# b0nefish/tiler

Hardware: AMD Instinct MI355X
Metric: FrameTiling Mtiles/sec @1080p 8×8, 64k tileset; % HBM roofline at 1/2/4/8 GPU (higher is better)
Workload: dtype f32

## Files before the change

include/tiler_ann.h:

```cpp
#ifndef TILER_ANN_H
#define TILER_ANN_H

#include <stdint.h>

#ifdef __cplusplus
extern "C" {
#endif

typedef struct ann_kdtree ann_kdtree;

ann_kdtree *ann_kdtree_create(float **pa, int n, int dd, int bs, int split);
void ann_kdtree_destroy(ann_kdtree *akd);
int ann_kdtree_search(ann_kdtree *akd, float *q, float eps, float *err);
int ann_kdtree_pri_search(ann_kdtree *akd, float *q, float eps, float *err);
int ann_kdtree_search_multi(ann_kdtree *akd, int *idxs, float *errs, int cnt, float *q, float eps);

#define TILER_SPLIT_ANN_KD_STD 0
#define TILER_SPLIT_INDEX_ORDER 100

ann_kdtree *ann_kdtree_create_dev(const float *d_rows, int n, int dd, void *stream);
ann_kdtree *ann_kdtree_create_dev_ex(const float *d_rows, int n, int dd, int bs, int split, void *stream);

int ann_kdtree_search_batch(ann_kdtree *akd, const float *q, int nq, float eps, int *idx, float *err);
int ann_kdtree_search_multi_batch(ann_kdtree *akd, const float *q, int nq, int k, float eps, int *idxs, float *errs);
int ann_kdtree_pri_search_batch(ann_kdtree *akd, const float *q, int nq, float eps, int *idx, float *err);
int ann_kdtree_search_batch_dev(ann_kdtree *akd, const float *d_q, int nq, int k, int *d_idx, float *d_err,
                                void *stream);

typedef struct {
    int64_t queries;
    int64_t fallback_queries;
    int64_t exhaustive_queries;
    int32_t exact_integer;
    int32_t splits;
    int64_t orbit_groups;
    int32_t orbit_search;
    int32_t orbit_ksteps;
    int64_t orbit_expansions;
    int64_t orbit_rescored;
    int32_t tie_order;
    int32_t kd_levels;
    double kd_build_ms;
    int64_t kd_replayed;
    int64_t flat_queries;
    int64_t searched_queries;
    int64_t searched_flat_queries;
    int64_t dup_queries;
} tiler_search_stats;
int ann_kdtree_get_stats(ann_kdtree *akd, tiler_search_stats *out);
int tiler_set_scan_limits(int max_k1, int max_k8);
int tiler_debug_force_replay(int on);
int tiler_debug_pri_outcomes(ann_kdtree *akd, int64_t out[3]);
int tiler_debug_shortlist_gate(int on);
int tiler_debug_ft_dedup(int mode);
int tiler_combine_stats(ann_kdtree *akd, int64_t *calls, int64_t *batches, int32_t *max_batch);
int tiler_debug_percall_bench(ann_kdtree *akd, const float *q, int nq, int k, int threads, int32_t *idx, float *err,
                              double *wall_s, double *lone_us);
int tiler_kdtree_positions(ann_kdtree *akd, int32_t *pos);

#define TILER_ALL_DEVICES (-1)
int tiler_init(int device);
int tiler_device_count(void);
int tiler_kdtree_device(ann_kdtree *akd);
int tiler_kdtree_replicate(ann_kdtree *akd, int device);
int tiler_placement_plan(int ndev, const int64_t *bytes, int n, int32_t *dev_out);
int tiler_debug_force_replicas(int on);
int tiler_shutdown(void);
const char *tiler_last_error(void);
int tiler_set_gamma(double g0, double g1);
int tiler_timing_enable(int on);
double tiler_timing_get(const char *kernel, int *launches);
int tiler_timing_reset(void);

int tiler_psyv_batch(int n, const int32_t *rgb, int n_tiles, const uint8_t *palpix, const int32_t *tile_of, int n_palettes,
                     const int32_t *palettes,
                     const int32_t *pal_of, const uint8_t *flags_per, int flags, int gamma, double *out64, float *out32);
int tiler_psyv_batch_dev(int n, const int32_t *rgb, const uint8_t *palpix, const int32_t *tile_of,
                         const int32_t *palettes, const int32_t *pal_of, const uint8_t *flags_per, int flags, int gamma,
                         double *out64, float *out32, void *stream);
int tiler_psyv_batch_ps(int n, const int32_t *rgb, int n_tiles, const uint8_t *palpix, const int32_t *tile_of,
                        int n_palettes, int palsize, const int32_t *palettes, const int32_t *pal_of,
                        const uint8_t *flags_per, int flags, int gamma, double *out64, float *out32);
int tiler_psyv_batch_ps_dev(int n, const int32_t *rgb, const uint8_t *palpix, const int32_t *tile_of,
                            const int32_t *palettes, int palsize, const int32_t *pal_of, const uint8_t *flags_per,
                            int flags, int gamma, double *out64, float *out32, void *stream);
int tiler_debug_psyv_lane_items(int64_t min_items);

// ... 268 lines not shown
```

tiler_amd/_lib.py:

```python
from __future__ import annotations

import ctypes
import os
import re

_HERE = os.path.dirname(os.path.abspath(__file__))
LIB_PATH = os.path.join(_HERE, "lib", "libANN.so")
_DEFAULT_LIB_PATH = LIB_PATH
HEADER_PATH = os.path.join(os.path.dirname(_HERE), "include", "tiler_ann.h")

c_int = ctypes.c_int
c_long = ctypes.c_long
c_float = ctypes.c_float
c_double = ctypes.c_double
c_void_p = ctypes.c_void_p
c_char_p = ctypes.c_char_p
c_size_t = ctypes.c_size_t
c_uint32 = ctypes.c_uint32
P = ctypes.POINTER


class TilerError(RuntimeError):
    pass

# ... 21 lines not shown
    _fields_ = [("tile", c_void_p), ("pal", c_void_p), ("hm", c_void_p), ("vm", c_void_p), ("smoothed", c_void_p),
                ("palpix", c_void_p), ("thm", c_void_p), ("tvm", c_void_p), ("palettes", c_void_p),
                ("kf_start", c_void_p), ("frames", ctypes.c_int64), ("positions", ctypes.c_int64),
                ("tiles", ctypes.c_int64), ("keyframes", ctypes.c_int32), ("n_palettes", ctypes.c_int32),
                ("palsize", ctypes.c_int32), ("first_keyframe", ctypes.c_int32), ("width", ctypes.c_int32),
                ("height", ctypes.c_int32), ("fps", c_double)]


class PrepareInfo(ctypes.Structure):
    _fields_ = [("items", ctypes.c_int64), ("candidates", ctypes.c_int64)]


_SIGS = {
    "ann_kdtree_create": (c_void_p, [P(P(c_float)), c_int, c_int, c_int, c_int]),
    "ann_kdtree_create_dev": (c_void_p, [c_void_p, c_int, c_int, c_void_p]),
    "ann_kdtree_create_dev_ex": (c_void_p, [c_void_p, c_int, c_int, c_int, c_int, c_void_p]),
    "tiler_kdtree_positions": (c_int, [c_void_p, c_void_p]),
    "ann_kdtree_destroy": (None, [c_void_p]),
    "ann_kdtree_search": (c_int, [c_void_p, c_void_p, c_float, c_void_p]),
    "ann_kdtree_pri_search": (c_int, [c_void_p, c_void_p, c_float, c_void_p]),
    "ann_kdtree_search_multi": (c_int, [c_void_p, c_void_p, c_void_p, c_int, c_void_p, c_float]),
    "ann_kdtree_search_batch": (c_int, [c_void_p, c_void_p, c_int, c_float, c_void_p, c_void_p]),
    "ann_kdtree_search_multi_batch": (c_int, [c_void_p, c_void_p, c_int, c_int, c_float, c_void_p, c_void_p]),
    "ann_kdtree_pri_search_batch": (c_int, [c_void_p, c_void_p, c_int, c_float, c_void_p, c_void_p]),
    "ann_kdtree_search_batch_dev": (c_int, [c_void_p, c_void_p, c_int, c_int, c_void_p, c_void_p, c_void_p]),
    "ann_kdtree_get_stats": (c_int, [c_void_p, P(SearchStats)]),
    "tiler_set_scan_limits": (c_int, [c_int, c_int]),
    "tiler_debug_percall_bench": (c_int, [c_void_p, c_void_p, c_int, c_int, c_int, c_void_p, c_void_p, P(c_double),
                                          P(c_double)]),
    "tiler_debug_force_replay": (c_int, [c_int]),
    "tiler_debug_pri_outcomes": (c_int, [c_void_p, P(ctypes.c_int64)]),
    "tiler_debug_shortlist_gate": (c_int, [c_int]),
    "tiler_debug_ft_dedup": (c_int, [c_int]),
    "tiler_combine_stats": (c_int, [c_void_p, P(ctypes.c_int64), P(ctypes.c_int64), P(ctypes.c_int32)]),
    "tiler_init": (c_int, [c_int]),
    "tiler_device_count": (c_int, []),
    "tiler_kdtree_device": (c_int, [c_void_p]),
    "tiler_kdtree_replicate": (c_int, [c_void_p, c_int]),
    "tiler_placement_plan": (c_int, [c_int, c_void_p, c_int, c_void_p]),
    "tiler_debug_force_replicas": (c_int, [c_int]),
    "tiler_shutdown": (c_int, []),
    "tiler_last_error": (c_char_p, []),
    "tiler_set_gamma": (c_int, [c_double, c_double]),
    "tiler_timing_enable": (c_int, [c_int]),
    "tiler_timing_get": (c_double, [c_char_p, P(c_int)]),
    "tiler_timing_reset": (c_int, []),
    "tiler_psyv_batch": (c_int, [c_int, c_void_p, c_int, c_void_p, c_void_p, c_int, c_void_p, c_void_p, c_void_p,
                                 c_int, c_int, c_void_p, c_void_p]),
    "tiler_psyv_batch_dev": (c_int, [c_int, c_void_p, c_void_p, c_void_p, c_void_p, c_void_p, c_void_p, c_int, c_int,
                                     c_void_p, c_void_p, c_void_p]),
    "tiler_psyv_batch_ps": (c_int, [c_int, c_void_p, c_int, c_void_p, c_void_p, c_int, c_int, c_void_p, c_void_p,
                                    c_void_p, c_int, c_int, c_void_p, c_void_p]),
    "tiler_psyv_batch_ps_dev": (c_int, [c_int, c_void_p, c_void_p, c_void_p, c_void_p, c_int, c_void_p, c_void_p,
                                        c_int, c_int, c_void_p, c_void_p, c_void_p]),
    "tiler_ft_set_maps": (c_int, [c_void_p, c_void_p, c_void_p, c_void_p]),
    "tiler_ft_get_maps": (c_int, [c_void_p, c_void_p, c_void_p, c_void_p]),
    "tiler_prepare_frame_tiling_dev": (c_void_p, [c_void_p, c_void_p, c_void_p, ctypes.c_int64, c_void_p, c_void_p,
                                                  c_void_p, c_int, c_void_p, c_int, c_int, c_void_p, c_int, c_int,
                                                  c_void_p, P(PrepareInfo)]),
    "tiler_prepare_frame_tiling_ps_dev": (c_void_p, [c_void_p, c_void_p, c_void_p, ctypes.c_int64, c_void_p,
                                                     c_void_p, c_void_p, c_int, c_void_p, c_int, c_int, c_int,
                                                     c_void_p, c_int, c_int, c_void_p, P(PrepareInfo)]),
    "tiler_frame_tiling": (c_int, [c_void_p, c_void_p, c_int, c_int, c_int, c_void_p, c_void_p, c_void_p, c_void_p,
                                   c_void_p]),
    "tiler_frame_tiling_dev": (c_int, [c_void_p, c_void_p, c_int, c_int, c_int, c_void_p, c_void_p, c_void_p,
                                       c_void_p, c_void_p, c_void_p]),
# ... 181 lines not shown
```

tiler_amd/csrc/ann_api.hip:

```cpp
#include <float.h>
#include <math.h>
#include <string.h>

#include <atomic>
#include <algorithm>
#include <chrono>
#include <thread>
#include <condition_variable>
#include <deque>
#include <mutex>
#include <string>
#include <vector>

#include "../../include/tiler_ann.h"
#include "dither.hpp"
#include "gtm_write.hpp"
#include "palette.hpp"
#include "play.hpp"
#include "prepare.hpp"
#include "kmeans.hpp"
#include "detmath.hpp"
#include "keyframes.hpp"
#include "load.hpp"
#include "scale.hpp"
// ... 950 lines not shown
int ann_kdtree_search_multi(ann_kdtree *t, int *idxs, float *errs, int cnt, float *q, float eps) {
    (void)eps;
    return combined_search(t, q, cnt, idxs, errs);
}

int tiler_set_scan_limits(int max_k1, int max_k8) {
    if (max_k1 < 0 || max_k8 < 0) {
        set_error("tiler_set_scan_limits: negative limit");
        return -1;
    }
    nn_set_scan_limits(max_k1, max_k8);
    return 0;
}

int tiler_debug_force_replay(int on) {
    nn_set_force_replay(on);
    return 0;
}

int tiler_debug_shortlist_gate(int on) {
    nn_set_shortlist_gate(on);
    return 0;
}

int tiler_debug_ft_dedup(int mode) {
    if (mode < 0 || mode > 2) {
        set_error("tiler_debug_ft_dedup: mode must be 0, 1 or 2");
        return -1;
    }
    nn_set_ft_dedup(mode);
    return 0;
}

int tiler_combine_stats(ann_kdtree *t, int64_t *calls, int64_t *batches, int32_t *max_batch) {
    if (!t) {
        set_error("tiler_combine_stats: null handle");
        return -1;
    }
    std::lock_guard<std::mutex> lk(t->comb.m);
    if (calls) *calls = t->comb.calls;
    if (batches) *batches = t->comb.batches;
    if (max_batch) *max_batch = t->comb.max_batch;
    return 0;
}

int tiler_debug_percall_bench(ann_kdtree *t, const float *q, int nq, int k, int threads, int32_t *idx, float *err,
                              double *wall_s, double *lone_us) {
    if (!t || !t->ix || nq < 0 || (nq > 0 && (!q || !idx || !err)) || k < 1 || k > 32 || threads < 1 || threads > 256) {
        set_error("tiler_debug_percall_bench: invalid arguments");
        return -1;
    }
    const int d = t->ix->d;
    auto call = [&](int i) -> int {
        float *qi = const_cast<float *>(q + (size_t)i * d);
        if (k == 1) {
            const int r = ann_kdtree_search(t, qi, 0.0f, err + i);
            idx[i] = r;
            return r < 0 && t->ix->n > 0 ? -1 : 0;
        }
        return ann_kdtree_search_multi(t, idx + (size_t)i * k, err + (size_t)i * k, k, qi, 0.0f);
    };
    const int nl = std::min(nq, 64);
    std::vector<double> lat;
    for (int i = 0; i < nl; i++) {
        const auto a = std::chrono::steady_clock::now();
        if (call(i)) return -1;
// ... 999 lines not shown
```

tiler_amd/csrc/frame_tiling.hip:

```cpp
#include "frame_tiling.hpp"

#include <atomic>

#include "nn_search.hpp"
#include "orbit.hpp"
#include "psyv.hpp"

namespace tiler {

__global__ __launch_bounds__(256) void ft_flat_flag_kernel(const int32_t *__restrict__ rgb, int Q, uint8_t *flag,
                                                           int *bcnt) {
    const long i = (long)blockIdx.x * 256 + threadIdx.x;
    int other = 0;
    if (i < Q) {
        const int4 *t = reinterpret_cast<const int4 *>(rgb + i * 64);
        const int c0 = rgb[i * 64];
        bool flat = true;
#pragma unroll
        for (int k = 0; k < 16; k++) {
            const int4 v = t[k];
            flat = flat && v.x == c0 && v.y == c0 && v.z == c0 && v.w == c0;
        }
        flag[i] = flat ? 1 : 0;
        other = flat ? 0 : 1;
// ... 264 lines not shown
            }
            TILER_HIP_CHECK(hipStreamSynchronize(stream));
            const int U = f.h_cnt[0] + f.h_cnt[1];
            if (U < 1 || U > Q) {
                set_error("frame tiling: inconsistent representative count");
                return -1;
            }
            engaged = U <= Q - Q / 8;
            if (engaged) {
                nq = U;
                rep_of = f.drep;
            } else if (group) {
                cnt = f.fcnt + 2;
                place(nullptr, f.fbcnt + (size_t)2 * nb, nullptr, cnt);
            }
        } else {
            hipLaunchKernelGGL(ft_flat_flag_kernel, dim3(nb), dim3(256), 0, stream, d_rgb, Q, f.fflag, f.fbcnt);
            hipLaunchKernelGGL(ft_flat_scan_kernel, dim3(1), dim3(1024), 0, stream, f.fbcnt, nb, f.fcnt);
            place(nullptr, f.fbcnt, nullptr, cnt);
        }
        TILER_HIP_CHECK(hipGetLastError());
        if (engaged || group) {
            perm = f.fperm;
            if (group) flat_cnt = cnt;
        }
    }

    FtMaps fm;
    if (maps) fm = perm ? FtMaps{f.ftile, f.fpal, f.fhm, f.fvm} : *maps;
    SearchOpts so;
    so.rootbox_ready = fuse_rb;
    so.orbit_prepared = orbit;
    so.flat_cnt = flat_cnt;
    const float *box = fuse_rb ? ix->kd->d_box : nullptr;
    float *rootbox = fuse_rb ? ix->scratch.kd_rootbox : nullptr;
    if (orbit) {
        if (orbit_ft_queries(ix, d_rgb, nq, gamma, f.qrows, box, rootbox, stream, perm)) return -1;
    } else {
        PsyvArgs pa;
        pa.n = nq;
        pa.rgb = d_rgb;
        pa.perm = perm;
        pa.flags = use_wavelets ? PSYV_WAVELETS : 0;
        pa.gamma = gamma;
        pa.out32 = f.qrows;
        pa.box = box;
        pa.rootbox = rootbox;
        if (launch_psyv(pa, stream)) return -1;
    }
    if (nn_search_dev(ix, f.qrows, nq, 1, perm ? f.fidx : d_idx, perm ? f.ferr : d_err, maps ? &fm : nullptr, stream, so))
        return -1;
    if (!perm) return 0;
    if (rep_of) {
        ix->last.queries = Q;
        ix->last.dup = Q - nq;
        ix->last.ft_nonflat = f.h_cnt[2];
    }
    KTimer tm(rep_of ? "ft_dedup" : nullptr, stream);
    hipLaunchKernelGGL(ft_output_kernel, dim3(nb), dim3(256), 0, stream, Q, rep_of, (const int *)f.dpos,
                       (const int *)f.fidx, (const float *)f.ferr, (const int32_t *)f.ftile, (const int32_t *)f.fpal,
                       (const uint8_t *)f.fhm, (const uint8_t *)f.fvm, d_idx, d_err, maps ? *maps : FtMaps{});
    TILER_HIP_CHECK(hipGetLastError());
    return 0;
}

}
// ... 1 lines not shown
```

tiler_amd/csrc/nn_search.hip:

```cpp
#include <float.h>
#include <math.h>
#include <stdlib.h>
#include <string.h>

#include <algorithm>
#include <atomic>

#include "nn_search.hpp"
#include "kdorder_dev.hpp"
#include "nn_dev.hpp"
#include "orbit.hpp"
#include "orbit_map_gen.hpp"

#pragma clang fp contract(off)

namespace tiler {

enum { QF_INT = 1, QF_BAD = 2 };

struct PrepArgs {
    const float *rows;
    long n;
    int d, S;
    float scale;
// ... 1726 lines not shown
    TILER_HIP_CHECK(hipGetLastError());
    return 0;
}

static int search_core(NNIndex *ix, RescoreArgs &ra, const float *d_q, int nq, int k, hipStream_t stream,
                       const SearchOpts &opt) {
    if (scan_small_takes(ix, nq, k)) return scan_small(ix, ra, nq, k, stream);
    const bool mfma = ix->S > 0 && k <= 8;
    if (!mfma) {
        ix->last.splits = 0;
        ix->last.fallback = nq;
        ra.tq.ex_list = nullptr;
        return launch_exact(ra, nq, std::min(nq, 4096), stream);
    }
    const int v16 = ix->S16 > 0 ? SL16_L : 0;
    const int L = v16 ? v16 : 8;
    const int lpq = v16 ? 4 : 2;
    const int nblk = v16 ? ix->nblk16 : ix->nblk;
    const int max_split = 64 / (lpq * L);
    const int qpwg = v16 ? SL16_NW * SL16_QB * 16 : (ix->S == 12 ? 512 : ix->S == 4 ? 32 * gen_qb_s4(nq) * GEN_NW_S4 : 256);
    const int wgs = (nq + qpwg - 1) / qpwg;
    int nsplit = std::max(1, std::min(max_split, (1024 + wgs - 1) / wgs));
    nsplit = std::min(nsplit, nblk);
    const int bps = (nblk + nsplit - 1) / nsplit;
    nsplit = (nblk + bps - 1) / bps;
    ix->last.splits = nsplit;
    if (ensure_scratch(ix, nq, (long)nq * nsplit * lpq * L)) return -1;
    SearchScratch &s = ix->scratch;
    TILER_HIP_CHECK(hipMemsetAsync(s.fb_count, 0, 16, stream));
    ix->last_orbit = 0;
    ra.tq = TierQueues{s.fb_list, s.fb_count, s.ex_list, s.fb_count + 1, nq, s.thr};
    ra.qstat = s.qstat;
    if (k == 1 && ix->orbit) {
        const OrbitTail t{ra.tq, ra.kd, ra.out, s.t2best, opt.flat_cnt, nullptr};
        if (orbit_search(ix, d_q, nq, t, stream, opt.orbit_prepared && k == 1)) return -1;
        ix->last_orbit = 1;
        return search_tail(ix, ra, nq, stream, &t);
    }
    const long nqblk = (nq + 31) / 32;
    PrepArgs pa{d_q, nq, ix->d, ix->S, ix->scale, (half8 *)s.qfrag, nullptr, nullptr, s.qstat, nullptr, 0};
    {
        KTimer t_prep("nn_prep", stream);
        hipLaunchKernelGGL(prep_rows_kernel, dim3((unsigned)std::min<long>(4096, (nqblk + 3) / 4)), dim3(256), 0,
                           stream, pa);
    }
    TILER_HIP_CHECK(hipGetLastError());
    if (v16) {
        Prep16Args p16{d_q, nq, ix->d, ix->S16, ix->scale, (half8 *)s.qfrag16, nullptr, 0, ix->d == 192 ? 1 : 0};
        {
            KTimer t_prep("nn_prep", stream);
            hipLaunchKernelGGL(prep16_kernel, dim3((unsigned)std::min<long>(4096, ((nq + 15) / 16 + 3) / 4)),
                               dim3(256), 0, stream, p16);
        }
        TILER_HIP_CHECK(hipGetLastError());
        {
            if (launch_shortlist16<6, SL16_L>(ix, nq, nsplit, bps, k == 1 && g_gate16.load(std::memory_order_relaxed),
                                         opt.flat_cnt, stream))
                return -1;
        }
    } else if (dispatch_shortlist<8>(ix, nq, nsplit, bps, stream)) {
        return -1;
    }
    ra.key = s.key;
    ra.idx = s.idx;
    ra.L = L;
    ra.lpq = lpq;
    ra.nsplit = nsplit;
// ... 42 lines not shown
```

tiler_amd/csrc/nn_search.hpp:

```cpp
#pragma once
#include <mutex>
#include <vector>

#include "frame_tiling.hpp"
#include "kdtree.hpp"
#include "tiler_common.hpp"

namespace tiler {

struct DsStat {
    unsigned long long max_n2_bits;
    unsigned long long max_h2_bits;
    unsigned long long max_e2_bits;
    unsigned long long max_abs_bits;
    unsigned int not_int;
    unsigned int bad;
    unsigned int pad[2];
};

struct QStat {
    double n2;
    double hn;
    double en;
    int flags;
// ... 6 lines not shown
    void *qfrag = nullptr;
    QStat *qstat = nullptr;
    float *key = nullptr;
    int *idx = nullptr;
    int *fb_list = nullptr;
    int *fb_count = nullptr;
    void *qfrag16 = nullptr;
    float *thr = nullptr;
    float2 *gate = nullptr;
    int *ex_list = nullptr;
    int *ccnt = nullptr;
    int *cbuf = nullptr;
    unsigned long long *t2best = nullptr;
    int *kd_list = nullptr;
    int *kd_count = nullptr;
    float *kd_rootbox = nullptr;
    uint8_t *kd_done = nullptr;
    size_t cap_q = 0, cap_keys = 0;
};

struct TierQueues {
    int *fb_list, *fb_count;
    int *ex_list, *ex_count;
    int fb_max;
    float *thr;
};

struct LastSearch {
    long long queries = 0, fallback = 0;
    int splits = 0;
    const int *flat_dev = nullptr;
    long flat_nq = 0, flat_qpw = 0, flat_wgs = 0;
    long long searched = 0, dup = 0, ft_nonflat = -1;
};

struct NNIndex {
    int n = 0, d = 0, S = 0, nblk = 0;
    float scale = 1.0f;
    double maxN = 0, maxH = 0, maxE = 0, max_abs = 0;
    bool exact_int = false;
    int perm = 0;
    float *d_rows = nullptr;
    float *d_rowsT = nullptr;
    void *d_frag = nullptr;
    float *d_nc = nullptr;
    float *d_seed = nullptr;
    int S16 = 0, nblk16 = 0;
    void *d_frag16 = nullptr;
    float *d_seed16 = nullptr;
    int32_t *d_tr_tile = nullptr, *d_tr_pal = nullptr;
    uint8_t *d_tr_attr = nullptr;
    SearchScratch scratch;
    std::mutex mu;
    LastSearch last;
    FtScratch ft;
    hipEvent_t done_event = nullptr;
    int last_orbit = 0;
    OrbitIndex *orbit = nullptr;
    KdTree *kd = nullptr;
    int bs = 1, split = KD_SPLIT_STD;
    int *h_fb_count = nullptr;
};

NNIndex *nn_index_create_dev(float *d_rows, int n, int d, int bs, int split, hipStream_t stream);
void nn_index_destroy(NNIndex *ix);
void nn_scratch_free(SearchScratch &s, bool synced = false);
bool nn_search_is_small(const NNIndex *ix, int nq, int k);

struct FtMaps {
    int32_t *tile = nullptr, *pal = nullptr;
    uint8_t *hm = nullptr, *vm = nullptr;
};

struct SearchOpts {
    bool rootbox_ready = false;
    bool orbit_prepared = false;
    const int *flat_cnt = nullptr;
    int *h_idx = nullptr;
    float *h_err = nullptr;
};

int nn_search_dev(NNIndex *ix, const float *d_q, int nq, int k, int *d_idx, float *d_err, const FtMaps *maps,
                  hipStream_t stream, const SearchOpts &opt = SearchOpts());
int nn_ensure_rootbox(NNIndex *ix, int nq);
bool nn_generic_takes_flat(const NNIndex *ix);

void nn_set_scan_limits(int max_k1, int max_k8);
void nn_set_force_replay(int on);
void nn_set_shortlist_gate(int on);

}
```

tiler_amd/csrc/orbit.hip:

```cpp
#include <float.h>
#include <math.h>
#include <string.h>

#include <algorithm>
#include <vector>

#include "kdorder_dev.hpp"
#include "nn_dev.hpp"
#include "psyv_dev.hpp"
#include "orbit.hpp"
#include "orbit_map_gen.hpp"

namespace tiler {

static constexpr int OD = 192;
static constexpr int OS = 12;
#ifndef ORB_XBATCH
#define ORB_XBATCH 3
#endif
#ifndef ORB_RS_WAVES
#define ORB_RS_WAVES 6
#endif
#ifndef ORB_STG_ROWS
#define ORB_STG_ROWS 4
#endif
#ifndef ORB_PR_UNROLL
#define ORB_PR_UNROLL 8
#endif
#ifndef ORB_DU
#define ORB_DU 4
#endif

struct OrbitMap {
    int16_t src[OD][4];
    float w[OD][4];
    float cs[OD], qs[OD];
    int16_t msrc[3][OD];
// ... 381 lines not shown
            t_bd |= bad;
        }
    }
    if (dataset) {
        __shared__ double r_d[ORB_PW][4];
        __shared__ int r_b[ORB_PW];
        const double mn = wave_max_d(t_n2), mp2 = wave_max_d(t_p2), mh = wave_max_d(t_h2), me = wave_max_d(t_e2);
        const int bd = __any(t_bd);
        if (lane == 0) {
            r_d[w][0] = mn;
            r_d[w][1] = mp2;
            r_d[w][2] = mh;
            r_d[w][3] = me;
            r_b[w] = bd;
        }
        __syncthreads();
        if (tid == 0) {
            double v[4] = {0.0, 0.0, 0.0, 0.0};
            int b = 0;
            for (int x = 0; x < ORB_PW; x++) {
                for (int y = 0; y < 4; y++) v[y] = fmax(v[y], r_d[x][y]);
                b |= r_b[x];
            }
            atomicMax(&a.ds->max_n2, (unsigned long long)__double_as_longlong(v[0]));
            atomicMax(&a.ds->max_p2, (unsigned long long)__double_as_longlong(v[1]));
            atomicMax(&a.ds->max_h2, (unsigned long long)__double_as_longlong(v[2]));
            atomicMax(&a.ds->max_e2, (unsigned long long)__double_as_longlong(v[3]));
            if (b) atomicOr(&a.ds->bad, 1u);
        }
    }
}

template <int L, int CB, int NW, int QB>
__global__ __launch_bounds__(NW * 64, 1) void nn_orbit_shortlist_pipe_kernel(const half8 *__restrict__ cfrag,
                                                                         const float *__restrict__ cseed, int nblk,
                                                                         const half8 *__restrict__ qfrag, int nq,
                                                                         int blk_per_split, int nsplit,
                                                                         float *__restrict__ out_key,
                                                                         int *__restrict__ out_id, int red_end,
                                                                         const uint8_t *__restrict__ bmask,
                                                                         const uint8_t *__restrict__ bmask0,
                                                                         const int *__restrict__ flat_cnt) {
    extern __shared__ __attribute__((aligned(16))) char smem[];
    constexpr int FRAG_BYTES = CB * OS * 1024;
    constexpr int BUF_BYTES = FRAG_BYTES + CB * 128;
    constexpr int NT = NW * 64;
    constexpr int PER_T = CB * OS * 64 / NT;
    static_assert((CB * OS * 64) % NT == 0, "stage must split evenly over the workgroup");
    static_assert(CB % 2 == 0, "accumulator roles alternate over pairs of blocks");
    const int tid = threadIdx.x, lane = tid & 63, w = tid >> 6, h = lane >> 5;
    const int nqblk = (nq + 31) / 32;
    const int qb0 = (blockIdx.x * NW + w) * QB;
    const int split = blockIdx.y;
    const int b_begin = split * blk_per_split;
    const int b_end = min(nblk, b_begin + blk_per_split);

    half8 bq[QB][OS];
#pragma unroll
    for (int q = 0; q < QB; q++) {
        const long qa = min(qb0 + q, nqblk - 1);
#pragma unroll
        for (int s = 0; s < OS; s++) bq[q][s] = qfrag[(qa * OS + s) * 64 + lane];
    }
    __builtin_amdgcn_s_waitcnt(0x0F70);
    float lk[QB][L], th[QB];
    int li[QB][L];
#pragma unroll
    for (int q = 0; q < QB; q++) {
        th[q] = -INFINITY;
#pragma unroll
        for (int i = 0; i < L; i++) {
            lk[q][i] = INFINITY;
            li[q][i] = -1;
        }
    }

    const int flat_wg0 = flat_cnt ? (max(0, *flat_cnt) + NW * QB * 32 - 1) / (NW * QB * 32) : 0x7fffffff;
    const bool flat = (int)blockIdx.x >= flat_wg0;
    const int nks = flat ? 3 : OS;
    if (flat) {
        red_end = nblk;
        bmask = bmask0;
    }
    const int r_end = max(b_begin, min(b_end, red_end));
    const int p_begin = r_end;
    auto issue_k3 = [&](int base, int end, int st, int buf) __attribute__((always_inline)) {
        const int blk0 = base + st * CB;
        const int nb = min(CB, end - blk0);
#pragma unroll
        for (int j = 0; j < (CB * 192 + NT - 1) / NT; j++) {
            const int e0 = j * NT + w * 64;
            if (e0 < CB * 192) {
                const int cb = e0 / 192, r0 = e0 % 192;
                const int cbc = min(cb, nb - 1);
                glds16_asm(reinterpret_cast<const uint4 *>(cfrag) + (long)(blk0 + cbc) * OS * 64 + r0 + lane,
                           smem + buf * BUF_BYTES + (cb * OS * 64 + r0) * 16);
            }
        }
        if (w == 0 && lane < CB * 8)
            glds16_asm(reinterpret_cast<const uint4 *>(cseed) + (long)blk0 * 8 + min(lane, nb * 8 - 1),
                       smem + buf * BUF_BYTES + FRAG_BYTES);
    };
    auto issue_rng = [&](int base, int end, int st, int buf) __attribute__((always_inline)) {
        const int blk0 = base + st * CB;
        const int nb = min(CB, end - blk0);
        const uint4 *src = reinterpret_cast<const uint4 *>(cfrag) + (long)blk0 * OS * 64 + w * 64 + lane;
        char *dst = smem + buf * BUF_BYTES + w * 1024;
        if (nb == CB) {
#pragma unroll
            for (int j = 0; j < PER_T; j++) glds16_asm(src + j * NT, dst + j * NT * 16);
        } else {
// ... 183 lines not shown
    for (int st = 0; st < nstage; st++) {
        const char *B = smem + (st & 1) * BUF_BYTES;
        const half8 *A = reinterpret_cast<const half8 *>(B) + lane;
        const float4 *SD = reinterpret_cast<const float4 *>(B + FRAG_BYTES) + h * 4;
        a0 = A[0];
        a1 = A[64];
        sd0 = SD[0];
        sd1 = SD[1];
        sd2 = SD[2];
        sd3 = SD[3];
        asm volatile("s_waitcnt lgkmcnt(0)" ::: "memory");
        if (st + 1 < nstage) issue(st + 1, (st + 1) & 1);
#pragma unroll
        for (int cb = 0; cb < CB; cb += 2) {
            body(A, SD, cb, p_begin + st * CB + cb, RA, RC);
            body(A, SD, cb + 1, p_begin + st * CB + cb + 1, RC, RA);
        }
        dma_drain();
        __syncthreads();
    }
    if (pend >= 0) {
#pragma unroll
        for (int q = 0; q < QB; q++) {
            float m4[4];
#pragma unroll
            for (int r = 0; r < 16; r++) RC[q][r] = RC[q][r] + fabsf(RB[q][r]);
            const float mx = maxima(RC[q], m4);
            if (__any(mx > th[q])) insert_block(q, m4, pend);
        }
    }
#pragma unroll
    for (int q = 0; q < QB; q++) {
        const int qq = (qb0 + q) * 32 + (lane & 31);
        if (qb0 + q < nqblk && qq < nq) {
            const long o = (((long)qq * nsplit + split) * 2 + h) * L;
#pragma unroll
            for (int i = 0; i < L; i++) {
                out_key[o + i] = lk[q][i];
                out_id[o + i] = li[q][i];
            }
        }
    }
}

struct OrbitRescoreArgs {
    const float *rows, *q;
    const _Float16 *rowh;
    const half8 *qfrag;
    const float *nc;
    const int *member;
    const uint8_t *dup;
    const uint8_t *rep;
    const GroupOrder *gorder;
    const int *grp_of;
    const OrbitStat *ostat;
    const float *key;
    const int *id;
    int G, nq, L, nsplit;
    int q0;
    int p1;
    int *pair_cnt;
    int *pair_cand;
    double scale2;
    double N, Np, Hp, Ecp;
    OrbitTail t;
};

__device__ __forceinline__ float exact_dist192_lean(const float *__restrict__ q, const float *__restrict__ c) {
    const float4 *q4 = reinterpret_cast<const float4 *>(q), *c4 = reinterpret_cast<const float4 *>(c);
    float dist = 0.0f;
#pragma unroll ORB_PR_UNROLL
    for (int i = 0; i < OD / 4; i++) {
        const float4 x = q4[i], y = c4[i];
        float t;
        t = x.x - y.x; dist = dist + t * t;
// ... 1028 lines not shown
            }
        if (ok) {
            const long nb = (G + 63) / 64;
            TILER_HIP_CHECK(dmalloc((void **)&o->d_base, (size_t)nb * 64 * OD * sizeof(float)));
            hipLaunchKernelGGL(orbit_base_kernel, dim3((unsigned)std::min<long>(8192, (nb * 64 * (OD / 4) + 255) / 256)),
                               dim3(256), 0, stream, ix->d_rows, (const int *)o->d_member, G, (float4 *)o->d_base);
            TILER_HIP_CHECK(hipGetLastError());
        }
    }
    {
        std::vector<uint8_t> ones(o->gblk, 1);
        TILER_HIP_CHECK(dmalloc((void **)&o->d_bmask0, o->gblk));
        TILER_HIP_CHECK(hipMemcpyAsync(o->d_bmask0, ones.data(), o->gblk, hipMemcpyHostToDevice, stream));
        TILER_HIP_CHECK(hipStreamSynchronize(stream));
    }
    ix->orbit = o;
    return 0;
}

static constexpr int ORB_L = 4, ORB_CB = 4, ORB_NW = 8, ORB_QB = 2;

int orbit_ensure_queries(OrbitIndex *o, int nq) {
    if ((size_t)nq <= o->cap_q) return 0;
    const long nqblk = (nq + 31) / 32;
    o->cap_q = 0;
    TILER_HIP_CHECK(dregrow({{o->pair_cnt, (size_t)nq * sizeof(int)},
                             {o->pair_cand, (size_t)nq * ORB_PSLOTS * sizeof(int)},
                             {o->qfrag, (size_t)(nqblk + 1) * OS * 1024},
                             {o->qstat, (size_t)nq * sizeof(OrbitStat)}}));
    o->cap_q = nq;
    return 0;
}

int orbit_search(NNIndex *ix, const float *d_q, int nq, const OrbitTail &tail, hipStream_t stream,
                 bool queries_prepared) {
    OrbitIndex *o = ix->orbit;
    const int nqblk = (nq + 31) / 32;
    const int qpw = ORB_NW * ORB_QB;
    const int wgs = (nqblk + qpw - 1) / qpw;
    const int max_split = 32 / (2 * ORB_L);
    static const int n_cu = [] {
        int dev = 0, cu = 256;
        if (hipGetDevice(&dev) == hipSuccess) (void)hipDeviceGetAttribute(&cu, hipDeviceAttributeMultiprocessorCount, dev);
        return cu > 0 ? cu : 256;
    }();
    constexpr double ORB_WG_FIXED = 64.0;
    int nsplit = 1;
    double best_t = 1e30;
    for (int ns = 1; ns <= max_split && ns <= o->gblk; ns++) {
        const double t = std::ceil((double)wgs * ns / n_cu) * (std::ceil((double)o->gblk / ns) + ORB_WG_FIXED);
        if (t < best_t * 0.98) {
            best_t = t;
            nsplit = ns;
        }
    }
    int mix_full = 0;
    {
        const int R = wgs / n_cu, rem = wgs - R * n_cu;
        for (int ns = 2; R >= 1 && rem > 0 && ns <= max_split && ns <= o->gblk; ns++) {
            const double t = R * (o->gblk + ORB_WG_FIXED) +
                             std::ceil((double)rem * ns / n_cu) * (std::ceil((double)o->gblk / ns) + ORB_WG_FIXED);
            if (t < best_t * 0.98) {
                best_t = t;
                nsplit = ns;
                mix_full = R * n_cu;
            }
        }
    }
    const int qpw_q = qpw * 32;
    const int *flat_cnt = tail.flat_cnt;
    if (flat_cnt) mix_full = 0;
    const int bps = (o->gblk + nsplit - 1) / nsplit;
    nsplit = (o->gblk + bps - 1) / bps;
    if (orbit_ensure_queries(o, nq)) return -1;
    const size_t nkeys = (size_t)nq * nsplit * 2 * ORB_L;
    if (nkeys > o->cap_keys) {
        o->cap_keys = 0;
        TILER_HIP_CHECK(dregrow({{o->key, nkeys * sizeof(float)}, {o->id, nkeys * sizeof(int)}}));
        o->cap_keys = nkeys;
    }
    if (!queries_prepared) {
        OrbitPrepArgs pa{d_q, nullptr, nq, (const OrbitMap *)o->d_map, ix->scale, (half8 *)o->qfrag,
                         nullptr, nullptr, nullptr, nullptr, o->qstat};
        KTimer tm("nn_prep", stream);
        hipLaunchKernelGGL(orbit_prep_kernel, dim3((unsigned)std::min<long>(4096, (nqblk + ORB_PW - 1) / ORB_PW)),
                           dim3(64 * ORB_PW), 0, stream, pa);
        TILER_HIP_CHECK(hipGetLastError());
    }
    {
        const size_t lds = 2 * ((size_t)ORB_CB * OS * 1024 + ORB_CB * 128);
        const size_t per_q = (size_t)nsplit * 2 * ORB_L;
        KTimer tm("nn_orbit", stream);
        auto shortlist = [&](int wg, int ns, int qb, int n, int blk, const int *fc) {
            hipLaunchKernelGGL((nn_orbit_shortlist_pipe_kernel<ORB_L, ORB_CB, ORB_NW, ORB_QB>), dim3(wg, ns),
                               dim3(ORB_NW * 64), lds, stream, (const half8 *)o->d_frag, o->d_seed, o->gblk,
                               (const half8 *)o->qfrag + (size_t)qb * OS * 64, n, blk, nsplit,
                               o->key + (size_t)qb * 32 * per_q, o->id + (size_t)qb * 32 * per_q, o->red_end,
                               o->d_bmask, o->d_bmask0, fc);
        };
        if (!mix_full) {
            shortlist(wgs, nsplit, 0, nq, bps, flat_cnt);
        } else {
            const int qb_off = mix_full * qpw, q_off = qb_off * 32;
            const size_t na = (size_t)std::min(nq, q_off) * per_q;
            TILER_HIP_CHECK(hipMemsetD32Async((hipDeviceptr_t)o->key, 0x7f800000u, na, stream));
            TILER_HIP_CHECK(hipMemsetAsync(o->id, 0xff, na * sizeof(int), stream));
            shortlist(mix_full, 1, 0, nq, o->gblk, nullptr);
            if (nq > q_off) shortlist(wgs - mix_full, nsplit, qb_off, nq - q_off, bps, nullptr);
        }
    }
    TILER_HIP_CHECK(hipGetLastError());
    OrbitRescoreArgs ra;
    ra.rows = ix->d_rows;
    ra.q = d_q;
    ra.rowh = (const _Float16 *)o->d_rowh;
    ra.qfrag = (const half8 *)o->qfrag;
    ra.nc = o->d_nc;
    ra.member = o->d_member;
    ra.dup = o->d_dup;
    ra.rep = o->d_rep;
    ra.gorder = tail.kd.ko ? o->d_gorder : nullptr;
    ra.grp_of = tail.kd.ko ? o->d_grp_of : nullptr;
    ra.ostat = o->qstat;
    ra.key = o->key;
    ra.id = o->id;
    ra.G = o->G;
    ra.nq = nq;
    ra.q0 = 0;
    ra.L = ORB_L;
    ra.nsplit = nsplit;
    ra.p1 = 2;
    ra.pair_cnt = o->pair_cnt;
    ra.pair_cand = o->pair_cand;
    ra.scale2 = (double)ix->scale * (double)ix->scale;
    ra.N = o->N;
    ra.Np = o->Np;
    ra.Hp = o->Hp;
    ra.Ecp = o->Ecp;
    ra.t = tail;
    static const bool want_stats = [] {
        const char *e = getenv("TILER_ORBIT_STATS");
        return e && e[0] == '1';
    }();
    if (want_stats) {
        if (!o->d_stats) TILER_HIP_CHECK(dmalloc((void **)&o->d_stats, 2 * sizeof(int)));
        TILER_HIP_CHECK(hipMemsetAsync(o->d_stats, 0, 2 * sizeof(int), stream));
        ra.t.n_expand = o->d_stats;
    }
    {
        KTimer tm("nn_rescore", stream);
        hipLaunchKernelGGL(nn_orbit_rescore_kernel, dim3((unsigned)((nq + 7) / 8)), dim3(256), 0, stream, ra);
    }
    TILER_HIP_CHECK(hipGetLastError());
    {
        static_assert(256 % ORB_PSLOTS == 0, "pair groups must not straddle blocks");
        KTimer tm("nn_pairs", stream);
        const long lanes = (long)nq * ORB_PSLOTS;
        hipLaunchKernelGGL(nn_orbit_pairs_kernel, dim3((unsigned)((lanes + 255) / 256)), dim3(256), 0, stream, ra);
    }
    TILER_HIP_CHECK(hipGetLastError());
    if (want_stats) {
        int h[2];
        TILER_HIP_CHECK(hipMemcpyAsync(h, o->d_stats, sizeof(h), hipMemcpyDeviceToHost, stream));
        TILER_HIP_CHECK(hipStreamSynchronize(stream));
        o->last_expansions = h[0];
        o->last_rescored = h[1];
    }
    ix->last.splits = nsplit;
    ix->last.flat_dev = flat_cnt;
    ix->last.flat_nq = nq;
    ix->last.flat_qpw = qpw_q;
    ix->last.flat_wgs = wgs;
    return 0;
}

void orbit_counters(const NNIndex *ix, long long *expansions, long long *rescored) {
    const OrbitIndex *o = ix->orbit;
    *expansions = o ? o->last_expansions : 0;
    *rescored = o ? o->last_rescored : 0;
}

}
```

tiler_amd/csrc/orbit.hpp:

```cpp
#pragma once
#include "nn_search.hpp"

namespace tiler {

struct OrbitStat {
    double n2;
    double hn;
    double en;
    int flags;
    int pad;
};

struct GroupOrder {
    uint16_t cd[3];
    uint16_t pad;
    float cv[3];
    uint32_t pairs;
};

struct OrbitIndex {
    int G = 0, gblk = 0;
    void *d_frag = nullptr;
    void *d_rowh = nullptr;
    float *d_seed = nullptr;
// ... 9 lines not shown
    int ksteps = 0;
    uint8_t *d_bmask = nullptr;
    uint8_t *d_bmask0 = nullptr;
    double N = 0, Np = 0, Hp = 0, Ecp = 0;
    void *qfrag = nullptr;
    OrbitStat *qstat = nullptr;
    int *pair_cnt = nullptr, *pair_cand = nullptr;
    size_t cap_q = 0;
    float *key = nullptr;
    int *id = nullptr;
    size_t cap_keys = 0;
    int *d_stats = nullptr;
    long long last_expansions = 0, last_rescored = 0;
};

__device__ __forceinline__ bool group_before(const GroupOrder *__restrict__ go, const float *__restrict__ q, int x,
                                             int y) {
    const int lo = min(x, y), hi = max(x, y);
    const int pi = lo == 0 ? hi - 1 : lo == 1 ? hi + 1 : 5;
    const unsigned code = (go->pairs >> (3 * pi)) & 7u;
    const int node = code & 3;
    const bool lo_first = (q[go->cd[node]] - go->cv[node]) < 0.0f;
    const bool low_slot_first = ((code >> 2) & 1) == (unsigned)lo_first;
    return (x == lo) == low_slot_first;
}

struct OrbitTail {
    TierQueues tq;
    KdCheck kd;
    ResultSink out;
    unsigned long long *t2_best;
    const int *flat_cnt;
    int *n_expand;
};

int orbit_build(NNIndex *ix, hipStream_t stream);
void orbit_destroy(OrbitIndex *o, bool synced = false);
inline long long orbit_groups(const NNIndex *ix) { return ix->orbit ? ((const OrbitIndex *)ix->orbit)->G : 0; }
inline int orbit_ksteps(const NNIndex *ix) { return ix->orbit ? ((const OrbitIndex *)ix->orbit)->ksteps : 0; }
void orbit_counters(const NNIndex *ix, long long *expansions, long long *rescored);
int orbit_search(NNIndex *ix, const float *d_q, int nq, const OrbitTail &tail, hipStream_t stream,
                 bool queries_prepared = false);
int orbit_ensure_queries(OrbitIndex *o, int nq);
int orbit_tier2(NNIndex *ix, const float *d_q, const OrbitTail &tail, int nq, hipStream_t stream);
int orbit_ft_queries(NNIndex *ix, const int32_t *d_rgb, int Q, int gamma, float *qrows, const float *box,
                     float *rootbox, hipStream_t stream, const int *perm = nullptr);

}
```

Baseline: 142.1.

## Level orbit shortlist tail with partial workgroups planned by makespan model

Adds a host-side planner that reshapes the orbit shortlist launch: some full workgroups (two query blocks per wave), some partial workgroups that give certain waves a single query block, then flat workgroups. A simple greedy makespan model over CU count picks the split to even out the final wave of work across CUs. The kernel body is templated on 1 or 2 query blocks per wave, and a host-known nonflat count is passed from frame tiling so the plan can run without a device readback. This adds code-size and instantiation cost, and the cost constants are heuristic.

```diff
diff --git a/include/tiler_ann.h b/include/tiler_ann.h
--- a/include/tiler_ann.h
+++ b/include/tiler_ann.h
@@ -53,6 +53,10 @@
 int tiler_debug_pri_outcomes(ann_kdtree *akd, int64_t out[3]);
 int tiler_debug_shortlist_gate(int on);
 int tiler_debug_ft_dedup(int mode);
+int tiler_debug_orbit_level(int blocks, int n_full, int n_cu);
+int tiler_debug_orbit_plan(int64_t nonflat, int64_t flat, int n_cu, int blocks, int n_full, int32_t out[4]);
+int tiler_debug_orbit_wave_blocks(const int32_t level[4], int nqblk, int wg, int wave, int32_t out[3]);
+int tiler_debug_orbit_last_level(ann_kdtree *akd, int32_t out[4]);
 int tiler_combine_stats(ann_kdtree *akd, int64_t *calls, int64_t *batches, int32_t *max_batch);
 int tiler_debug_percall_bench(ann_kdtree *akd, const float *q, int nq, int k, int threads, int32_t *idx, float *err,
                               double *wall_s, double *lone_us);
diff --git a/tiler_amd/_lib.py b/tiler_amd/_lib.py
--- a/tiler_amd/_lib.py
+++ b/tiler_amd/_lib.py
@@ -77,6 +77,10 @@
     "tiler_debug_pri_outcomes": (c_int, [c_void_p, P(ctypes.c_int64)]),
     "tiler_debug_shortlist_gate": (c_int, [c_int]),
     "tiler_debug_ft_dedup": (c_int, [c_int]),
+    "tiler_debug_orbit_level": (c_int, [c_int, c_int, c_int]),
+    "tiler_debug_orbit_plan": (c_int, [ctypes.c_int64, ctypes.c_int64, c_int, c_int, c_int, P(ctypes.c_int32)]),
+    "tiler_debug_orbit_wave_blocks": (c_int, [P(ctypes.c_int32), c_int, c_int, c_int, P(ctypes.c_int32)]),
+    "tiler_debug_orbit_last_level": (c_int, [c_void_p, P(ctypes.c_int32)]),
     "tiler_combine_stats": (c_int, [c_void_p, P(ctypes.c_int64), P(ctypes.c_int64), P(ctypes.c_int32)]),
     "tiler_init": (c_int, [c_int]),
     "tiler_device_count": (c_int, []),
diff --git a/tiler_amd/csrc/ann_api.hip b/tiler_amd/csrc/ann_api.hip
--- a/tiler_amd/csrc/ann_api.hip
+++ b/tiler_amd/csrc/ann_api.hip
@@ -1006,6 +1006,54 @@
     return 0;
 }
 
+int tiler_debug_orbit_level(int blocks, int n_full, int n_cu) {
+    if ((blocks != 0 && (blocks < 8 || blocks > 16)) || n_full < 0 || n_cu < 0) {
+        set_error("tiler_debug_orbit_level: blocks must be 0 or 8..16, n_full and n_cu >= 0");
+        return -1;
+    }
+    orbit_set_level(blocks, n_full, n_cu);
+    return 0;
+}
+
+int tiler_debug_orbit_plan(int64_t nonflat, int64_t flat, int n_cu, int blocks, int n_full, int32_t out[4]) {
+    if (!out || nonflat < 0 || flat < 0 || nonflat + flat > 0x7fffffff || n_cu < 1 ||
+        (blocks != 0 && (blocks < 8 || blocks > 16)) || n_full < 0) {
+        set_error("tiler_debug_orbit_plan: invalid arguments");
+        return -1;
+    }
+    const OrbitLevel lv = orbit_level_plan((long)nonflat, (long)flat, n_cu, blocks, n_full);
+    out[0] = lv.n_full;
+    out[1] = lv.n_part;
+    out[2] = lv.part;
+    out[3] = lv.flat_qb0;
+    return 0;
+}
+
+int tiler_debug_orbit_wave_blocks(const int32_t level[4], int nqblk, int wg, int wave, int32_t out[3]) {
+    if (!level || !out || nqblk < 0 || wg < 0 || wave < 0 || wave > 7 || level[0] < 0 || level[1] < 0 ||
+        level[2] < 8 || level[2] > 16 || level[3] < 0) {
+        set_error("tiler_debug_orbit_wave_blocks: invalid arguments");
+        return -1;
+    }
+    const OrbitLevel lv{level[0], level[1], level[2], level[3]};
+    int qb0 = 0;
+    bool flat = false;
+    out[1] = orbit_wave_blocks(lv, 8, nqblk, wg, wave, &qb0, &flat);
+    out[0] = qb0;
+    out[2] = flat ? 1 : 0;
+    return 0;
+}
+
+int tiler_debug_orbit_last_level(ann_kdtree *t, int32_t out[4]) {
+    if (!t || !t->ix || !out) {
+        set_error("tiler_debug_orbit_last_level: invalid arguments");
+        return -1;
+    }
+    std::lock_guard<std::mutex> lk(t->ix->mu);
+    for (int i = 0; i < 4; i++) out[i] = t->ix->last.level[i];
+    return 0;
+}
+
 int tiler_combine_stats(ann_kdtree *t, int64_t *calls, int64_t *batches, int32_t *max_batch) {
     if (!t) {
         set_error("tiler_combine_stats: null handle");
diff --git a/tiler_amd/csrc/frame_tiling.hip b/tiler_amd/csrc/frame_tiling.hip
--- a/tiler_amd/csrc/frame_tiling.hip
+++ b/tiler_amd/csrc/frame_tiling.hip
@@ -320,6 +320,7 @@
     so.rootbox_ready = fuse_rb;
     so.orbit_prepared = orbit;
     so.flat_cnt = flat_cnt;
+    if (rep_of) so.host_nonflat = f.h_cnt[0];
     const float *box = fuse_rb ? ix->kd->d_box : nullptr;
     float *rootbox = fuse_rb ? ix->scratch.kd_rootbox : nullptr;
     if (orbit) {
diff --git a/tiler_amd/csrc/nn_search.hip b/tiler_amd/csrc/nn_search.hip
--- a/tiler_amd/csrc/nn_search.hip
+++ b/tiler_amd/csrc/nn_search.hip
@@ -1782,7 +1782,7 @@
     ra.tq = TierQueues{s.fb_list, s.fb_count, s.ex_list, s.fb_count + 1, nq, s.thr};
     ra.qstat = s.qstat;
     if (k == 1 && ix->orbit) {
-        const OrbitTail t{ra.tq, ra.kd, ra.out, s.t2best, opt.flat_cnt, nullptr};
+        const OrbitTail t{ra.tq, ra.kd, ra.out, s.t2best, opt.flat_cnt, nullptr, opt.host_nonflat};
         if (orbit_search(ix, d_q, nq, t, stream, opt.orbit_prepared && k == 1)) return -1;
         ix->last_orbit = 1;
         return search_tail(ix, ra, nq, stream, &t);
diff --git a/tiler_amd/csrc/nn_search.hpp b/tiler_amd/csrc/nn_search.hpp
--- a/tiler_amd/csrc/nn_search.hpp
+++ b/tiler_amd/csrc/nn_search.hpp
@@ -62,6 +62,7 @@
     const int *flat_dev = nullptr;
     long flat_nq = 0, flat_qpw = 0, flat_wgs = 0;
     long long searched = 0, dup = 0, ft_nonflat = -1;
+    int level[4] = {0, 0, 0, 0};
 };
 
 struct NNIndex {
@@ -106,6 +107,7 @@
     bool rootbox_ready = false;
     bool orbit_prepared = false;
     const int *flat_cnt = nullptr;
+    int host_nonflat = -1;
     int *h_idx = nullptr;
     float *h_err = nullptr;
 };
diff --git a/tiler_amd/csrc/orbit.hip b/tiler_amd/csrc/orbit.hip
--- a/tiler_amd/csrc/orbit.hip
+++ b/tiler_amd/csrc/orbit.hip
@@ -3,6 +3,8 @@
 #include <string.h>
 
 #include <algorithm>
+#include <atomic>
+#include <utility>
 #include <vector>
 
 #include "kdorder_dev.hpp"
@@ -450,15 +452,13 @@
 }
 
 template <int L, int CB, int NW, int QB>
-__global__ __launch_bounds__(NW * 64, 1) void nn_orbit_shortlist_pipe_kernel(const half8 *__restrict__ cfrag,
-                                                                         const float *__restrict__ cseed, int nblk,
-                                                                         const half8 *__restrict__ qfrag, int nq,
-                                                                         int blk_per_split, int nsplit,
-                                                                         float *__restrict__ out_key,
-                                                                         int *__restrict__ out_id, int red_end,
-                                                                         const uint8_t *__restrict__ bmask,
-                                                                         const uint8_t *__restrict__ bmask0,
-                                                                         const int *__restrict__ flat_cnt) {
+__device__ __forceinline__ void orbit_shortlist_wave(const half8 *__restrict__ cfrag, const float *__restrict__ cseed,
+                                                     int nblk, const half8 *__restrict__ qfrag, int nq,
+                                                     int blk_per_split, int nsplit, float *__restrict__ out_key,
+                                                     int *__restrict__ out_id, int red_end,
+                                                     const uint8_t *__restrict__ bmask,
+                                                     const uint8_t *__restrict__ bmask0, const int qb0, const int nown,
+                                                     const bool flat) {
     extern __shared__ __attribute__((aligned(16))) char smem[];
     constexpr int FRAG_BYTES = CB * OS * 1024;
     constexpr int BUF_BYTES = FRAG_BYTES + CB * 128;
@@ -468,7 +468,6 @@
     static_assert(CB % 2 == 0, "accumulator roles alternate over pairs of blocks");
     const int tid = threadIdx.x, lane = tid & 63, w = tid >> 6, h = lane >> 5;
     const int nqblk = (nq + 31) / 32;
-    const int qb0 = (blockIdx.x * NW + w) * QB;
     const int split = blockIdx.y;
     const int b_begin = split * blk_per_split;
     const int b_end = min(nblk, b_begin + blk_per_split);
@@ -493,8 +492,6 @@
         }
     }
 
-    const int flat_wg0 = flat_cnt ? (max(0, *flat_cnt) + NW * QB * 32 - 1) / (NW * QB * 32) : 0x7fffffff;
-    const bool flat = (int)blockIdx.x >= flat_wg0;
     const int nks = flat ? 3 : OS;
     if (flat) {
         red_end = nblk;
@@ -744,7 +741,7 @@
 #pragma unroll
     for (int q = 0; q < QB; q++) {
         const int qq = (qb0 + q) * 32 + (lane & 31);
-        if (qb0 + q < nqblk && qq < nq) {
+        if (q < nown && qq < nq) {
             const long o = (((long)qq * nsplit + split) * 2 + h) * L;
 #pragma unroll
             for (int i = 0; i < L; i++) {
@@ -753,6 +750,35 @@
             }
         }
     }
+}
+
+template <int L, int CB, int NW, int QB>
+__global__ __launch_bounds__(NW * 64, 1) void nn_orbit_shortlist_pipe_kernel(const half8 *__restrict__ cfrag,
+                                                                         const float *__restrict__ cseed, int nblk,
+                                                                         const half8 *__restrict__ qfrag, int nq,
+                                                                         int blk_per_split, int nsplit,
+                                                                         float *__restrict__ out_key,
+                                                                         int *__restrict__ out_id, int red_end,
+                                                                         const uint8_t *__restrict__ bmask,
+                                                                         const uint8_t *__restrict__ bmask0,
+                                                                         const int *__restrict__ flat_cnt,
+                                                                         OrbitLevel lv) {
+    static_assert(QB == 2, "orbit_wave_blocks gives a wave one or two query blocks");
+    if (lv.flat_qb0 < 0) {
+        lv.n_full = (max(0, *flat_cnt) + NW * QB * 32 - 1) / (NW * QB * 32);
+        lv.n_part = 0;
+        lv.flat_qb0 = lv.n_full * NW * QB;
+    }
+    const int w = __builtin_amdgcn_readfirstlane((int)threadIdx.x >> 6);
+    int qb0;
+    bool flat;
+    const int nown = orbit_wave_blocks(lv, NW, (nq + 31) / 32, (int)blockIdx.x, w, &qb0, &flat);
+    if (nown == 2)
+        orbit_shortlist_wave<L, CB, NW, 2>(cfrag, cseed, nblk, qfrag, nq, blk_per_split, nsplit, out_key, out_id, red_end,
+                                           bmask, bmask0, qb0, nown, flat);
+    else
+        orbit_shortlist_wave<L, CB, NW, 1>(cfrag, cseed, nblk, qfrag, nq, blk_per_split, nsplit, out_key, out_id, red_end,
+                                           bmask, bmask0, qb0, nown, flat);
 }
 
 struct OrbitRescoreArgs {
@@ -1847,6 +1873,69 @@
     return 0;
 }
 
+static constexpr int ORB_PART = 12;
+static constexpr double ORB_COST_PART = 0.80;
+static constexpr double ORB_COST_FLAT = 0.25;
+
+static std::atomic<int> g_level_blocks{0}, g_level_full{0}, g_level_cu{0};
+void orbit_set_level(int blocks, int n_full, int n_cu) {
+    g_level_blocks.store(blocks);
+    g_level_full.store(n_full);
+    g_level_cu.store(n_cu);
+}
+
+static double orbit_makespan(const long (&n)[3], const double (&c)[3], int n_cu) {
+    std::vector<std::pair<double, long>> free_at{{0.0, (long)n_cu}};
+    double end = 0.0;
+    for (int i = 0; i < 3; i++)
+        for (long m = n[i]; m > 0;) {
+            size_t g = 0;
+            for (size_t j = 1; j < free_at.size(); j++)
+                if (free_at[j].first < free_at[g].first) g = j;
+            const long k = std::min(m, free_at[g].second);
+            const double t = free_at[g].first + c[i];
+            end = std::max(end, t);
+            if (k == free_at[g].second)
+                free_at[g].first = t;
+            else {
+                free_at[g].second -= k;
+                free_at.push_back({t, k});
+            }
+            m -= k;
+        }
+    return end;
+}
+
+OrbitLevel orbit_level_plan(long nonflat, long flat, int n_cu, int blocks, int n_full) {
+    const long F = (nonflat + 31) / 32, nqblk = (nonflat + flat + 31) / 32;
+    const long nflat = (nqblk - F + 15) / 16;
+    const long single = (F + 15) / 16;
+    OrbitLevel lv{(int)single, 0, ORB_PART, (int)F};
+    if (blocks >= 8 && blocks < 16) {
+        lv.part = blocks;
+        lv.n_full = (int)std::min<long>(std::max(0, n_full), F / 16);
+        lv.n_part = (int)((F - 16L * lv.n_full + blocks - 1) / blocks);
+        return lv;
+    }
+    if (blocks == 16 || n_cu < 1) return lv;
+    const double cost[3] = {1.0, ORB_COST_PART, ORB_COST_FLAT};
+    const long n1[3] = {single, 0, nflat};
+    double best = orbit_makespan(n1, cost, n_cu) * 0.98;
+    const long R = F / 16 / n_cu;
+    for (long k = R; k >= 0 && k >= R - 1; k--) {
+        const long nf = k * n_cu, np = (F - 16 * nf + ORB_PART - 1) / ORB_PART;
+        if (np == 0) continue;
+        const long n2[3] = {nf, np, nflat};
+        const double t = orbit_makespan(n2, cost, n_cu);
+        if (t < best) {
+            best = t;
+            lv.n_full = (int)nf;
+            lv.n_part = (int)np;
+        }
+    }
+    return lv;
+}
+
 int orbit_search(NNIndex *ix, const float *d_q, int nq, const OrbitTail &tail, hipStream_t stream,
                  bool queries_prepared) {
     OrbitIndex *o = ix->orbit;
@@ -1854,11 +1943,13 @@
     const int qpw = ORB_NW * ORB_QB;
     const int wgs = (nqblk + qpw - 1) / qpw;
     const int max_split = 32 / (2 * ORB_L);
-    static const int n_cu = [] {
+    static const int dev_cu = [] {
         int dev = 0, cu = 256;
         if (hipGetDevice(&dev) == hipSuccess) (void)hipDeviceGetAttribute(&cu, hipDeviceAttributeMultiprocessorCount, dev);
         return cu > 0 ? cu : 256;
     }();
+    const int dbg_cu = g_level_cu.load(std::memory_order_relaxed);
+    const int n_cu = dbg_cu > 0 ? dbg_cu : dev_cu;
     constexpr double ORB_WG_FIXED = 64.0;
     int nsplit = 1;
     double best_t = 1e30;
@@ -1887,6 +1978,17 @@
     if (flat_cnt) mix_full = 0;
     const int bps = (o->gblk + nsplit - 1) / nsplit;
     nsplit = (o->gblk + bps - 1) / bps;
+    OrbitLevel level = ORB_LEVEL_NONE;
+    if (flat_cnt) level.flat_qb0 = -1;
+    if (tail.host_nonflat >= 0 && tail.host_nonflat <= nq && nsplit == 1 && !mix_full) {
+        const long nonflat = flat_cnt ? tail.host_nonflat : nq;
+        const OrbitLevel lv = orbit_level_plan(nonflat, nq - nonflat, n_cu,
+                                               g_level_blocks.load(std::memory_order_relaxed),
+                                               g_level_full.load(std::memory_order_relaxed));
+        if (lv.n_part > 0) level = lv;
+    }
+    const bool levelled = level.n_part > 0;
+    const int wgs_launch = levelled ? level.n_full + level.n_part + ((nqblk - level.flat_qb0 + qpw - 1) / qpw) : wgs;
     if (orbit_ensure_queries(o, nq)) return -1;
     const size_t nkeys = (size_t)nq * nsplit * 2 * ORB_L;
     if (nkeys > o->cap_keys) {
@@ -1906,22 +2008,22 @@
         const size_t lds = 2 * ((size_t)ORB_CB * OS * 1024 + ORB_CB * 128);
         const size_t per_q = (size_t)nsplit * 2 * ORB_L;
         KTimer tm("nn_orbit", stream);
-        auto shortlist = [&](int wg, int ns, int qb, int n, int blk, const int *fc) {
+        auto shortlist = [&](int wg, int ns, int qb, int n, int blk, const int *fc, const OrbitLevel &lv) {
             hipLaunchKernelGGL((nn_orbit_shortlist_pipe_kernel<ORB_L, ORB_CB, ORB_NW, ORB_QB>), dim3(wg, ns),
                                dim3(ORB_NW * 64), lds, stream, (const half8 *)o->d_frag, o->d_seed, o->gblk,
                                (const half8 *)o->qfrag + (size_t)qb * OS * 64, n, blk, nsplit,
                                o->key + (size_t)qb * 32 * per_q, o->id + (size_t)qb * 32 * per_q, o->red_end,
-                               o->d_bmask, o->d_bmask0, fc);
+                               o->d_bmask, o->d_bmask0, fc, lv);
         };
         if (!mix_full) {
-            shortlist(wgs, nsplit, 0, nq, bps, flat_cnt);
+            shortlist(wgs_launch, nsplit, 0, nq, bps, flat_cnt, level);
         } else {
             const int qb_off = mix_full * qpw, q_off = qb_off * 32;
             const size_t na = (size_t)std::min(nq, q_off) * per_q;
             TILER_HIP_CHECK(hipMemsetD32Async((hipDeviceptr_t)o->key, 0x7f800000u, na, stream));
             TILER_HIP_CHECK(hipMemsetAsync(o->id, 0xff, na * sizeof(int), stream));
-            shortlist(mix_full, 1, 0, nq, o->gblk, nullptr);
-            if (nq > q_off) shortlist(wgs - mix_full, nsplit, qb_off, nq - q_off, bps, nullptr);
+            shortlist(mix_full, 1, 0, nq, o->gblk, nullptr, ORB_LEVEL_NONE);
+            if (nq > q_off) shortlist(wgs - mix_full, nsplit, qb_off, nq - q_off, bps, nullptr, ORB_LEVEL_NONE);
         }
     }
     TILER_HIP_CHECK(hipGetLastError());
@@ -1986,6 +2088,12 @@
     ix->last.flat_nq = nq;
     ix->last.flat_qpw = qpw_q;
     ix->last.flat_wgs = wgs;
+    if (levelled) {
+        ix->last.level[0] = level.n_full;
+        ix->last.level[1] = level.n_part;
+        ix->last.level[2] = level.part;
+        ix->last.level[3] = level.flat_qb0;
+    }
     return 0;
 }
 
diff --git a/tiler_amd/csrc/orbit.hpp b/tiler_amd/csrc/orbit.hpp
--- a/tiler_amd/csrc/orbit.hpp
+++ b/tiler_amd/csrc/orbit.hpp
@@ -65,7 +65,38 @@
     unsigned long long *t2_best;
     const int *flat_cnt;
     int *n_expand;
+    int host_nonflat = -1;
 };
+
+struct OrbitLevel {
+    int n_full;
+    int n_part;
+    int part;
+    int flat_qb0;
+};
+static constexpr OrbitLevel ORB_LEVEL_NONE{0x7fffffff, 0, 0, 0x3fffffff};
+
+__host__ __device__ inline int orbit_wave_blocks(const OrbitLevel &lv, int nw, int nqblk, int wg, int w, int *qb0,
+                                                 bool *flat) {
+    int two = 1, lim = lv.flat_qb0 < nqblk ? lv.flat_qb0 : nqblk;
+    *flat = false;
+    if (wg < lv.n_full) {
+        *qb0 = (wg * nw + w) * 2;
+    } else if (wg < lv.n_full + lv.n_part) {
+        const int k = lv.part - nw;
+        two = w < k;
+        *qb0 = lv.n_full * nw * 2 + (wg - lv.n_full) * lv.part + (two ? 2 * w : w + k);
+    } else {
+        *flat = true;
+        lim = nqblk;
+        *qb0 = lv.flat_qb0 + ((wg - lv.n_full - lv.n_part) * nw + w) * 2;
+    }
+    const int left = lim - *qb0, want = two ? 2 : 1;
+    return left < 0 ? 0 : left < want ? left : want;
+}
+
+OrbitLevel orbit_level_plan(long nonflat, long flat, int n_cu, int blocks, int n_full);
+void orbit_set_level(int blocks, int n_full, int n_cu);
 
 int orbit_build(NNIndex *ix, hipStream_t stream);
 void orbit_destroy(OrbitIndex *o, bool synced = false);
```

Result: slower. 133.3 (-6.2%).
